# Zain-Jiang/Dict-TTS

Measured on AMD Instinct MI355X. Metric: mel-frames/sec, end-to-end text->mel->wav (audio-samples/sec = 256x; RTF reported alongside), higher is better.
Workload: dtype f16 (vocoder ResBlocks fp16 MFMA, serial convolutions bf16 hi/lo split; acoustic model fp32-grade: fp32 MFMA / bf16 three-piece operands x 6 products)

## Files before the change

dict_tts_amd/csrc/rb_common.h:

```cpp
#pragma once
#include <hip/hip_runtime.h>
#include <stdint.h>
#include "voc_el.h"

namespace dtts {

constexpr int VP_ST_AUX = 18;
constexpr int VP_LD_AUX = 18;
constexpr int VP_XI_AUX = 2;
constexpr int RB_X_AUX = 0;

typedef __attribute__((ext_vector_type(8))) __bf16 bf16x8;
typedef __attribute__((ext_vector_type(16))) float f32x16;
typedef __attribute__((ext_vector_type(4))) float f32x4;

__device__ __forceinline__ unsigned rf2bf(float f) {
    const __bf16 h = (__bf16)f;
    return (unsigned)__builtin_bit_cast(unsigned short, h);
}

typedef __attribute__((ext_vector_type(2))) float f32x2_t;
typedef __attribute__((ext_vector_type(2))) __bf16 bf16x2_t;
__device__ __forceinline__ unsigned pack2bf(float a, float b) {
    const bf16x2_t v = __builtin_convertvector(f32x2_t{a, b}, bf16x2_t);
// ... 226 lines not shown
            } else {
                xb += TU * dilP;
            }
        } else {
#pragma unroll
            for (int m = 0; m < MH * MT; ++m)
#pragma unroll
                for (int n = 0; n < NT; ++n) acc[m][n] = (*cinit)[n];
        }
    }
    for (; s0 < SG; s0 += 4) {
        const acc_t(&dummy)[NT] = *(const acc_t(*)[NT])acc[0];
        rb_group<EL, MT, NT, NKG, PITCH, false, MH, SH>(acc, dummy, ring, xa, act, wpf, xb, dilP, g);
        wpf += 4 * KGS;
        if constexpr (NKG >= 4) {
            if (++g == GPT) {
                g = 0;
                xb += dilP;
            }
        } else {
            xb += TU * dilP;
        }
    }
    if constexpr (TAIL) {
        const acc_t(&dummy)[NT] = *(const acc_t(*)[NT])acc[0];
        rb_group<EL, MT, NT, NKG, PITCH, false, MH, SH, 2>(acc, dummy, ring, xa, act, wpf, xb, dilP, 0);
    }
}

template <int NT, int RD>
__device__ __forceinline__ void rb2_preload(uint4 (&ring)[RD][NT], const uint4* w, int kgs) {
#pragma unroll
    for (int s = 0; s < RD - 1; ++s)
#pragma unroll
        for (int n = 0; n < NT; ++n) ring[s][n] = w[(size_t)s * kgs + n * 64];
}

template <int EL, int MT, int NT, int NKG, int PITCH, int RD, bool FIRST, bool CINIT>
__device__ __forceinline__ bool rb2_group(f32x16 (&acc)[MT][NT], const f32x16 (&cinit)[NT], uint4 (&ring)[RD][NT], uint4 (&xa)[MT],
                                          const char* act, const uint4* wpf, int xb, int dilP, int left) {
    constexpr int KGS = (NKG / 2) * 64;
    static_assert(RD % NKG == 0 && RD % 2 == 0, "a ring turn covers whole taps");
#pragma unroll
    for (int u = 0; u < RD; ++u) {
        if (u && u % NKG == 0 && u >= left) return true;
#pragma unroll
        for (int n = 0; n < NT; ++n) ring[(u + RD - 1) % RD][n] = wpf[u * KGS + n * 64];
        const int off = xb + ((u + 1) / NKG) * dilP + ((u + 1) % NKG) * 32;
        __builtin_amdgcn_sched_barrier(0);
#pragma unroll
        for (int m = 0; m < MT; ++m)
#pragma unroll
            for (int n = 0; n < NT; ++n) {
                if (FIRST && CINIT && u == 0) acc[m][n] = mfma16<EL>(ring[u][n], xa[m], cinit[n]);
                else acc[m][n] = mfma16<EL>(ring[u][n], xa[m], acc[m][n]);
                if (n == NT - 1) {
                    __builtin_amdgcn_sched_barrier(0);
                    xa[m] = *(const uint4*)(act + off + m * 32 * PITCH);
                    __builtin_amdgcn_sched_barrier(0);
                }
            }
        __builtin_amdgcn_sched_barrier(0);
    }
    return left <= RD;
}

template <int EL, int MT, int NT, int NKG, int PITCH, int RD, bool CINIT>
__device__ __forceinline__ void rb2_contract(f32x16 (&acc)[MT][NT], uint4 (&ring)[RD][NT], const char* act, int xrow0, const uint4* w, int S,
                                             int dilP, const f32x16 (&cinit)[NT]) {
    constexpr int KGS = (NKG / 2) * 64;
    uint4 xa[MT];
#pragma unroll
    for (int m = 0; m < MT; ++m) xa[m] = *(const uint4*)(act + xrow0 + m * 32 * PITCH);
    const uint4* wpf = w + (RD - 1) * KGS;
    int xb = xrow0;
    if (rb2_group<EL, MT, NT, NKG, PITCH, RD, true, CINIT>(acc, cinit, ring, xa, act, wpf, xb, dilP, S)) return;
    for (int left = S - RD;; left -= RD) {
        wpf += RD * KGS;
        xb += (RD / NKG) * dilP;
        if (rb2_group<EL, MT, NT, NKG, PITCH, RD, false, CINIT>(acc, cinit, ring, xa, act, wpf, xb, dilP, left)) return;
    }
}

}
```

dict_tts_amd/csrc/rblock.h:

```cpp
#pragma once
#include <hip/hip_runtime.h>
#include <stdint.h>
#include "voc_el.h"

namespace dtts {

struct RBlockParams {
    const float* x;
    float* S;
    unsigned short* Sa;
    struct Set {
        const uint4* w1[3];
        const uint4* w2[3];
        const float* b1[3];
        const float* b2[3];
        int dil[3];
        int K, Kp;
    } rb[3];
    int nrb;
    const int* lens;
    int B, T;
    int K;
    int mode;
    int last_mode;
    int drop_S;
    float div, slope;
    float* wav;
    const float* post_w;
    const float* post_b;
    int el;
    unsigned* tile_ctr;
    int pre_off;
    unsigned* bad;
    unsigned long long* ovf;
    int small_tile;
    int : 32;
    int s_private;
};

__host__ __device__ inline int rblock_halo_of(int K, const int* dil) {
    const int need = (K - 1) / 2 * (dil[0] + dil[1] + dil[2] + 3);
    return need > 6 * (K - 1) ? need : 6 * (K - 1);
}
__host__ __device__ inline int rblock_halo(const RBlockParams& p) {
    int h = 6 * (p.K - 1);
    for (int j = 0; j < p.nrb && j < 3; ++j) {
        const int need = rblock_halo_of(p.rb[j].K, p.rb[j].dil);
        h = need > h ? need : h;
    }
    return h;
}

constexpr int rblock_mfma_shape(int C) { return C == 64 ? 16 : 32; }

bool rblock_supported(int C, int K);
int rblock_padded_taps(int C, int K);
hipError_t rblock_launch(const RBlockParams& p, int C, int frag, hipStream_t stream);
long long rblock_private_rows(int C, int halo, int B, int T);
int rblock_stage_tile_rows(int C, int halo);
bool rblock_stage_launch_fits(int C, int halo, int B, bool wav);

}
```

dict_tts_amd/csrc/rblock.hip:

```cpp
#include "rblock.h"
#include "rb_common.h"

#include <algorithm>
#include <type_traits>
#include <cstdlib>

namespace dtts {

#ifdef RB_STAMP
__device__ unsigned long long rb_stamps[2][12][16];
extern "C" __attribute__((visibility("default"))) int dtts_debug_rb_stamps(unsigned long long* host, int reset) {
    hipError_t e = hipMemcpyFromSymbol(host, HIP_SYMBOL(rb_stamps), sizeof(rb_stamps));
    if (e == hipSuccess && reset) {
        static unsigned long long z[2][12][16];
        e = hipMemcpyToSymbol(HIP_SYMBOL(rb_stamps), z, sizeof z);
    }
    return (int)e;
}
#define RB_T(k) do { const unsigned long long _n = __builtin_amdgcn_s_memrealtime(); tq[k] += _n - t_last; t_last = _n; } while (0)
#else
#define RB_T(k)
#endif

template <int C, int MT, int NT, int WT, int WC, int EL, int PS, bool GUARD, bool TB = false, class SH = MfmaShape<32>>
// ... 53 lines not shown
    constexpr int RPP = THREADS / F4;
    constexpr int PER = SROWS / RPP;
    static_assert(THREADS % F4 == 0 && SROWS % RPP == 0, "row-coalesced staging");
    int c4 = tid % F4, r0 = tid / F4;
    auto tile_row = [&](int m, int u) { const int sr = r0 + RPP * u; return ((sr >> 5) * MT + m) * 32 + (sr & 31); };

    auto locate = [&](int jj, int& bb) {
        while (pre[bb + 1] <= jj) ++bb;
        bb = __builtin_amdgcn_readfirstlane(bb);
    };
    auto load_x = [&](acc_t (&d)[NT], int m, int bb, int base, int ln) {
        const auto rs = __builtin_amdgcn_make_buffer_rsrc((void*)(p.x + (long long)bb * p.T * C), 0, ln * C * 4, 0x00020000);
        const int o0 = ((base + wt * MT * 32 + SH::row(lane, 0)) * C + wc * NT * 32 + SH::chan(lane, 0)) * 4;
#pragma unroll
        for (int n = 0; n < NT; ++n)
#pragma unroll
            for (int q = 0; q < 4; ++q) {
                const u32x4 v = __builtin_amdgcn_raw_buffer_load_b128(rs, o0 + (m * 32 * C + n * 32 + SH::row(0, q) * C + SH::chan(0, q)) * 4, 0, RB_X_AUX);
                SH::set_quad(d[n], q, __builtin_bit_cast(f32x4, v));
            }
    };
    auto len_of = [&](int bb) { return __builtin_amdgcn_readfirstlane(pre[2 * p.B + 1 + bb]); };

    int b = 0, len, t0;
    if constexpr (PS) {
        locate(j, b);
        len = len_of(b);
        t0 = (j - pre[b]) * TTo - (p.wav ? PH : 0);
    } else {
        b = blockIdx.y;
        len = __builtin_amdgcn_readfirstlane(p.lens ? p.lens[b] : p.T);
        t0 = blockIdx.x * TTo - (p.wav ? PH : 0);
        if (t0 + (p.wav ? PH : 0) >= len) return;
    }
    acc_t xr[MT][NT];
    if constexpr (PS) {
#pragma unroll
        for (int m = 0; m < MT; ++m) load_x(xr[m], m, b, t0 - H, len);
    } else {
        const auto rs_x = __builtin_amdgcn_make_buffer_rsrc((void*)(p.x + (long long)b * p.T * C), 0, len * C * 4, 0x00020000);
        const int g0 = ((t0 - H + r0) * C + c4 * 4) * 4;
        u32x4 ld[MT][PER] = {};
#pragma unroll
        for (int m = 0; m < MT; ++m)
#pragma unroll
            for (int u = 0; u < PER; ++u) ld[m][u] = __builtin_amdgcn_raw_buffer_load_b128(rs_x, g0 + (tile_row(m, u) - r0) * (C * 4), 0, RB_X_AUX);
#pragma unroll
        for (int m = 0; m < MT; ++m) {
            if (m) __syncthreads();
#pragma unroll
            for (int u = 0; u < PER; ++u) *(u32x4*)(stage + (r0 + RPP * u) * EP + c4 * 16) = ld[m][u];
            __syncthreads();
#pragma unroll
            for (int n = 0; n < NT; ++n)
#pragma unroll
                for (int q = 0; q < 4; ++q)
                    SH::set_quad(xr[m][n], q, *(const f32x4*)(stage + (wt * 32 + SH::row(lane, q)) * EP + ((wc * NT + n) * 32 + SH::chan(lane, q)) * 4));
        }
    }

    const int kg_stride = (C / 32) * SH::WF * 64;
    int r = 0;

#ifdef RB_STAMP
    unsigned long long tq[16] = {0, 0, 0, 0, 0, 0, 0, 0, 0, 0, 0, 0, 0, 0, 0, 0};
    unsigned long long t_last = __builtin_amdgcn_s_memrealtime();
#endif
#pragma unroll 1
    for (;;) {
    if constexpr (PS) {
        tid = threadIdx.x;
        asm volatile("" : "+v"(tid));
        lane = tid & 63, wave = __builtin_amdgcn_readfirstlane(tid >> 6);
        wt = wave % WT, wc = wave / WT;
        c4 = tid % F4, r0 = tid / F4;
    }
    const int xlane = (RB_GUARD + wt * MT * 32 + SH::row(lane, 0)) * PITCH + SH::chan(lane, 0) * 4;
    const size_t wlane = (size_t)(wc * NT) * SH::WF * 64 + lane;
    if constexpr (PS) r = __builtin_amdgcn_readfirstlane(r);
    else r = 0;
    const RBlockParams::Set& R = p.rb[PS ? r : 0];
    const int Kr = R.K;
    constexpr bool REAL_STEPS = (C == 32);
    static_assert(!REAL_STEPS || SH::FRAG == 32, "rb2_contract is written for 32x32x16");
    static_assert(REAL_STEPS || NKG >= 4 || (NKG == 2 && SH::FRAG == 16), "whole groups of four k-steps, or rb_contract's half group");
    const int S = (REAL_STEPS ? Kr : R.Kp) * NKG;
    const bool last_rb = !PS || r + 1 == p.nrb;
    const int mode = (!PS || p.nrb == 1 || r == 0) ? p.mode : (last_rb ? p.last_mode : 1);
    const bool wav_now = p.wav && last_rb;
    t0 = __builtin_amdgcn_readfirstlane(t0);
    const int base_t = t0 - H;
    const long long brow = (long long)b * p.T;
    unsigned claim = 0;
    if (PS && p.tile_ctr && tid == 0 && last_rb) claim = atomicAdd(p.tile_ctr, 1u);
    int jn = j + G;
    bool has_next = PS && jn < total;
    int bn = b, lenn = len, t0n = 0;
    auto plan_next = [&]() {
        if (!last_rb) {
            has_next = true;
            jn = j;
            bn = b;
            lenn = len;
            t0n = t0;
            return;
        }
        has_next = PS && jn < total;
        bn = b;
        if (has_next) {
            locate(jn, bn);
            lenn = len_of(bn);
            t0n = (jn - pre[bn]) * TTo - (p.wav ? PH : 0);
        }
    };
    if (!(PS && p.tile_ctr) || !last_rb) plan_next();
    const auto rs_s = p.s_private ? __builtin_amdgcn_make_buffer_rsrc((void*)p.S, 0, p.s_private, 0x00020000)
                                  : __builtin_amdgcn_make_buffer_rsrc((void*)(p.S + brow * C), 0, len * C * 4, 0x00020000);

    constexpr int NBQ = 4 / SH::QB;
    auto load_bias = [&](f32x4 (&bb)[NT][NBQ], const float* bias) {
#pragma unroll
        for (int n = 0; n < NT; ++n)
#pragma unroll
            for (int q = 0; q < NBQ; ++q) bb[n][q] = *(const f32x4*)(bias + (wc * NT + n) * 32 + SH::chan(lane, q * SH::QB));
    };
    const bool all_inb = base_t >= 0 && base_t + W <= len;
    int n_ovf = 0;
    auto write_act_impl = [&](char* dst, const acc_t (&v)[MT][NT], auto masked_tag) {
        constexpr bool MASKED = decltype(masked_tag)::value;
        int ln = lane;
        if constexpr (SH::FRAG == 16) asm volatile("" : "+v"(ln));
#pragma unroll
        for (int m = 0; m < MT; ++m) {
            int row[SH::QB];
            bool inb[SH::QB], counted[SH::QB];
#pragma unroll
            for (int rh = 0; rh < SH::QB; ++rh) {
                row[rh] = (wt * MT + m) * 32 + SH::row(ln, rh);
                const int t = base_t + row[rh];
                inb[rh] = !MASKED || (t >= 0 && t < len);
                counted[rh] = inb[rh] && row[rh] >= H && row[rh] < H + TT;
            }
#pragma unroll
            for (int n = 0; n < NT; ++n)
#pragma unroll
                for (int q = 0; q < 4; ++q) {
                    constexpr int QBM = SH::QB - 1;
                    const int co = (wc * NT + n) * 32 + SH::chan(ln, q);
                    const f32x4 v4 = SH::quad(v[m][n], q);
                    uint2 pk = act4<EL>(v4, 0.1f);
                    if constexpr (GUARD) n_ovf += counted[q & QBM] ? ovf4(v4, 0.1f) : 0;
                    if constexpr (MASKED) {
                        if (!inb[q & QBM]) pk = make_uint2(0, 0);
                    }
                    *(uint2*)(dst + (RB_GUARD + row[q & QBM]) * PITCH + co * 2) = pk;
                }
        }
    };
    auto write_act = [&](char* dst, const acc_t (&v)[MT][NT]) {
        if (all_inb) write_act_impl(dst, v, std::false_type{});
        else write_act_impl(dst, v, std::true_type{});
    };

    uint4 ring[SH::RD][NT * SH::WF];
    f32x4 bb[NT][NBQ];
    RB_T(10);
    rb_preload(ring, R.w1[0] + wlane, kg_stride);
    load_bias(bb, R.b1[0]);
    write_act(act, xr);
    RB_T(0);
    __syncthreads();
    RB_T(1);

    acc_t acc[MT][NT];
#pragma unroll 1
    for (int it = 0; it < 3; ++it) {
        acc_t cinit[NT];
#pragma unroll
        for (int n = 0; n < NT; ++n)
#pragma unroll
            for (int q = 0; q < 4; ++q) SH::set_quad(cinit[n], q, bb[n][q / SH::QB]);
        load_bias(bb, R.b2[it]);
        const int d = R.dil[it];
        if constexpr (REAL_STEPS) {
            if (S) rb2_contract<EL, MT, NT, NKG, PITCH, 4, true>(acc, ring, act, xlane - ((Kr - 1) / 2) * d * PITCH, R.w1[it] + wlane, S, d * PITCH, cinit);
            else rb_contract<EL, MT, NT, NKG, PITCH, true, 1>(acc, ring, act, 0, R.w1[it] + wlane, 0, 0, &cinit);
        } else
            rb_contract<EL, MT, NT, NKG, PITCH, true, 1, SH>(acc, ring, act, xlane - ((Kr - 1) / 2) * d * PITCH, R.w1[it] + wlane, S, d * PITCH, &cinit);
        rb_preload(ring, R.w2[it] + wlane, kg_stride);
        RB_T(2);
        if constexpr (!TB) __syncthreads();
        RB_T(3);
        write_act(act2, acc);
        RB_T(4);
        __syncthreads();
        RB_T(5);
#pragma unroll
        for (int m = 0; m < MT; ++m)
#pragma unroll
            for (int n = 0; n < NT; ++n)
#pragma unroll
                for (int q = 0; q < 4; ++q) SH::add_quad(xr[m][n], q, bb[n][q / SH::QB]);
        if (it < 2) load_bias(bb, R.b1[it + 1]);
        if constexpr (REAL_STEPS) {
            if (S) rb2_contract<EL, MT, NT, NKG, PITCH, 4, false>(xr, ring, act2, xlane - ((Kr - 1) / 2) * PITCH, R.w2[it] + wlane, S, PITCH, cinit);
        } else
            rb_contract<EL, MT, NT, NKG, PITCH, false, 1, SH>(xr, ring, act2, xlane - ((Kr - 1) / 2) * PITCH, R.w2[it] + wlane, S, PITCH);
        if (it < 2) rb_preload(ring, R.w1[it + 1] + wlane, kg_stride);
        if (PS && p.tile_ctr && last_rb && it == 2 && tid == 0) pre[3 * p.B + 1] = G + (int)claim;
        RB_T(6);
        if (!TB || it == 2) __syncthreads();
        RB_T(7);
        if (it < 2) {
            write_act(act, xr);
            RB_T(0);
            __syncthreads();
            RB_T(1);
        }
    }

    if (PS && p.tile_ctr && last_rb) {
        jn = __builtin_amdgcn_readfirstlane(pre[3 * p.B + 1]);
        plan_next();
    }
    {
    const auto rs_a = __builtin_amdgcn_make_buffer_rsrc((void*)(p.Sa ? p.Sa + brow * C : (unsigned short*)(p.S + brow * C)), 0,
                                                        len * C * 2, 0x00020000);
    constexpr int CW = NT * 32, F4W = CW / 4, RPI = 64 / F4W, NRD = 32 / RPI;
    const int er = lane / F4W, ec = lane % F4W;
    const int goffw = (p.s_private ? (j * TT - H) * C : base_t * C) * 4 + (wc * CW + ec * 4) * 4;
    static_assert(F4W == 8 && RPI == 8 && NRD == 4, "the conflict-free row order below is for 8 lanes per row, 8 rows per access");
    const int erow_slab_base = C == 32 ? er : (er >> 2) + ((er & 1) ? 16 : 0) + ((er & 2) ? 8 : 0);
    auto srow = [&](int u) { return (C == 32 ? 8 : 2) * u + erow_slab_base; };
    auto erow = [&](int m, int u) { return (wt * MT + m) * 32 + srow(u); };
    auto eoff = [&](int m, int u) {
        const int row = erow(m, u);
        return (row >= H && row < H + TT) ? goffw + row * (C * 4) : (int)0x80000000;
    };
    u32x4 sold[MT][NRD];
#pragma unroll
    for (int m = 0; m < MT; ++m)
#pragma unroll
        for (int u = 0; u < NRD; ++u) {
            sold[m][u] = u32x4{0u, 0u, 0u, 0u};
            if (mode >= 1) sold[m][u] = p.nrb > 1 ? __builtin_amdgcn_raw_buffer_load_b128(rs_s, eoff(m, u), 0, 0)
                                                  : __builtin_amdgcn_raw_buffer_load_b128(rs_s, eoff(m, u), 0, VP_LD_AUX);
        }
    RB_T(12);
    constexpr int OP = C * 4;
    char* otile = smem;
    char* estage = wav_now ? smem + ((TB || (size_t)TT * OP > ACT_BYTES) ? (size_t)TT * OP : ACT_BYTES) : stage;
    char* stg = estage + (wt * 32) * EP + (wc * CW) * 4;
#pragma unroll
    for (int m = 0; m < MT; ++m) {
#pragma unroll
        for (int n = 0; n < NT; ++n)
#pragma unroll
            for (int q = 0; q < 4; ++q) *(f32x4*)(stg + SH::row(lane, q) * EP + (n * 32 + SH::chan(lane, q)) * 4) = SH::quad(xr[m][n], q);
        if (has_next) load_x(xr[m], m, bn, t0n - H, lenn);
        __builtin_amdgcn_fence(__ATOMIC_RELEASE, "wavefront");
        __builtin_amdgcn_wave_barrier();
        __builtin_amdgcn_fence(__ATOMIC_ACQUIRE, "wavefront");
        RB_T(13);
#pragma unroll
        for (int u = 0; u < NRD; ++u) {
            const int off = eoff(m, u);
            f32x4 o = *(const f32x4*)(stg + srow(u) * EP + ec * 16);
            o += __builtin_bit_cast(f32x4, sold[m][u]);
            if (wav_now) {
                const int row = erow(m, u);
                if (row >= H && row < H + TT) {
                    const int t = base_t + row;
#pragma unroll
                    for (int e = 0; e < 4; ++e) o[e] = (t >= 0 && t < len) ? lrelu(o[e] / p.div, p.slope) : 0.f;
                    *(f32x4*)(otile + (size_t)(row - H) * OP + (wc * CW + ec * 4) * 4) = o;
                }
                continue;
            }
            if (mode == 2) {
#pragma unroll
                for (int e = 0; e < 4; ++e) o[e] = o[e] / p.div;
            }
            if (!(mode == 2 && p.Sa && p.drop_S)) {
                if (p.nrb > 1 && !last_rb) __builtin_amdgcn_raw_buffer_store_b128(__builtin_bit_cast(u32x4, o), rs_s, off, 0, 0);
                else __builtin_amdgcn_raw_buffer_store_b128(__builtin_bit_cast(u32x4, o), rs_s, off, 0, VP_ST_AUX);
            }
            if (mode == 2 && p.Sa) {
// ... 97 lines not shown
static size_t rb_lds_bytes(int TT, bool wav) {
    constexpr int W = 32 * MT * WT, PITCH = C * 2 + 16, EP = C * 4 + 16;
    constexpr size_t ACT = (size_t)(W + 2 * RB_GUARD) * PITCH;
    if (wav)
        return TB ? std::max(2 * ACT, (size_t)TT * C * 4 + (size_t)WT * 32 * EP) : std::max((size_t)TT * C * 4, ACT) + (size_t)WT * 32 * EP;
    return TB ? std::max(2 * ACT, ACT + (size_t)RB_GUARD * PITCH + (size_t)WT * 32 * EP) : ACT + (size_t)WT * 32 * EP;
}
static size_t rb_table_bytes(int B) { return (size_t)(3 * B + 2) * sizeof(int); }

template <int C, int MT, int NT, int WT, int WC, int EL, int PS, bool GUARD = false, bool TB = false>
static hipError_t rb_launch_cfg(const RBlockParams& p, hipStream_t stream) {
    typedef MfmaShape<rblock_mfma_shape(C)> SH;
    constexpr int W = 32 * MT * WT;
    for (int j = 0; j < p.nrb; ++j)
        if (!(p.rb[j].K & 1) || p.rb[j].Kp != rblock_padded_taps(C, p.rb[j].K)) return hipErrorInvalidValue;
    const int H = rblock_halo(p), TT = W - 2 * H;
    if (TT < 32) return hipErrorInvalidValue;
    if ((long long)p.T * C * 4 >= (1LL << 31)) return hipErrorInvalidValue;
    if (p.wav && (C != 32 || (p.nrb == 1 && p.mode != 2) || !p.post_w || !p.post_b)) return hipErrorInvalidValue;
    size_t lds = rb_lds_bytes<C, MT, WT, TB>(TT, p.wav != nullptr);
    const int TTo = p.wav ? TT - 6 : TT;
    RBlockParams q = p;
    q.pre_off = (int)lds;
    if (PS) lds += rb_table_bytes(p.B);
    if (lds > 160 * 1024) return hipErrorOutOfMemory;
    constexpr bool HAS_GUARD = !(C == 64 && MT == 5);
    if constexpr (EL == EL_F16 && !GUARD && HAS_GUARD) {
        if (p.ovf) return rb_launch_cfg<C, MT, NT, WT, WC, EL, PS, true, TB>(p, stream);
    }
    if (EL == EL_F16 && !HAS_GUARD && p.ovf) return hipErrorInvalidValue;
    auto kern = rblock_kernel<C, MT, NT, WT, WC, EL, PS, GUARD, TB, SH>;
    static bool configured_dev[64] = {};
    int cur_dev = 0;
    (void)hipGetDevice(&cur_dev);
    bool& configured = configured_dev[cur_dev & 63];
    if (!configured) {
        hipError_t e = hipFuncSetAttribute((const void*)kern, hipFuncAttributeMaxDynamicSharedMemorySize, 160 * 1024);
        if (e != hipSuccess) return e;
        configured = true;
    }
    constexpr int THREADS = 64 * WT * WC;
    if (!PS) {
        hipLaunchKernelGGL(kern, dim3((p.T + TTo - 1) / TTo, p.B), dim3(THREADS), lds, stream, q);
        return hipGetLastError();
    }
    static int cus_dev[64] = {};
    int& cus = cus_dev[cur_dev & 63];
    if (!cus) {
        hipDeviceProp_t prop;
        if (hipGetDeviceProperties(&prop, cur_dev) != hipSuccess) return hipErrorInvalidDevice;
        cus = prop.multiProcessorCount;
    }
    const int per_cu = std::max(1, std::min({(int)(160 * 1024 / lds), 2048 / THREADS, THREADS <= 256 ? 2 : 1}));
    const long long max_tiles = (long long)p.B * ((p.T + TTo - 1) / TTo);
    const int grid = (int)std::min<long long>((long long)cus * per_cu, max_tiles);
    if (grid <= 0) return hipSuccess;
    hipLaunchKernelGGL(kern, dim3(grid), dim3(THREADS), lds, stream, q);
    return hipGetLastError();
}

bool rblock_supported(int C, int K) {
    if (!(K & 1) || K < 3 || K > 11) return false;
    return C == 32 || C == 64 || ((C == 128 || C == 256) && K == 3);
}

int rblock_stage_tile_rows(int C, int halo) {
    return (C == 32 ? 1024 : 512) - 2 * halo;
}

bool rblock_stage_launch_fits(int C, int halo, int B, bool wav) {
    const int TT = rblock_stage_tile_rows(C, halo);
    if (C != 32 && C != 64) return false;
    const size_t lds = (C == 32 ? rb_lds_bytes<32, 4, 8, false>(TT, wav) : rb_lds_bytes<64, 4, 4, false>(TT, wav)) + rb_table_bytes(B);
    return TT >= 32 && lds <= 160 * 1024;
}

long long rblock_private_rows(int C, int halo, int B, int T) {
    if (C != 32) return 0;
    const int TT = rblock_stage_tile_rows(C, halo), TTo = TT - 6;
    if (TTo < 32) return 0;
    return (long long)B * ((T + TTo - 1) / TTo) * TT;
}

int rblock_padded_taps(int C, int K) {
    const int sh = rblock_mfma_shape(C);
    const int nkg = C / (sh == 16 ? 32 : 16);
    if (sh == 16 && nkg == 2) return K;
    int kp = K;
    while ((kp * nkg) % 4) ++kp;
    return kp;
}

template <int EL>
static hipError_t rb_launch_el(const RBlockParams& p, int C, hipStream_t stream) {
    static int cus_dev[64] = {};
    int cur_dev = 0;
    (void)hipGetDevice(&cur_dev);
    int& cus = cus_dev[cur_dev & 63];
    if (!cus) {
        hipDeviceProp_t prop;
        cus = hipGetDeviceProperties(&prop, cur_dev) == hipSuccess ? prop.multiProcessorCount : 256;
    }
    auto few = [&](int W) {
        const int tt = W - 2 * rblock_halo(p) - (p.wav ? 6 : 0);
        return tt >= 32 && 2 * (long long)p.B * ((p.T + tt - 1) / tt) <= cus;
    };
    if (p.nrb < 1 || p.nrb > 3) return hipErrorInvalidValue;
    if (p.nrb > 1) {
        if (C == 32) return rb_launch_cfg<32, 4, 1, 8, 1, EL, 1>(p, stream);
        if (C == 64) return rb_launch_cfg<64, 4, 1, 4, 2, EL, 1>(p, stream);
        return hipErrorInvalidValue;
    }
#define RB_TRY(call)                                   \
    do {                                               \
        const hipError_t e_ = (call);                  \
        if (e_ != hipErrorOutOfMemory) return e_;      \
    } while (0)
    if (C == 32 && p.K >= 7 && !few(1024)) RB_TRY((rb_launch_cfg<32, 4, 1, 8, 1, EL, 1>(p, stream)));
    if (C == 64 && few(512)) return rb_launch_cfg<64, 4, 1, 2, 2, EL, 1>(p, stream);
    if (C == 128 && few(256)) return rb_launch_cfg<128, 4, 1, 1, 4, EL, 1>(p, stream);
    if (C == 256 && few(128)) return rb_launch_cfg<256, 2, 1, 1, 8, EL, 1>(p, stream);
    if (C == 32) return rb_launch_cfg<32, 4, 1, 4, 1, EL, 0>(p, stream);
    if (C == 64 && p.K >= 7 && !p.small_tile && !(EL == EL_F16 && p.ovf)) RB_TRY((rb_launch_cfg<64, 5, 1, 4, 2, EL, 1>(p, stream)));
    if (C == 64) RB_TRY((rb_launch_cfg<64, 4, 1, 4, 2, EL, 1>(p, stream)));
    if (C == 64) return rb_launch_cfg<64, 4, 1, 2, 2, EL, 1>(p, stream);
    if (C == 128) RB_TRY((rb_launch_cfg<128, 4, 1, 2, 4, EL, 1>(p, stream)));
    if (C == 128) return rb_launch_cfg<128, 4, 1, 1, 4, EL, 1>(p, stream);
    if (C == 256) RB_TRY((rb_launch_cfg<256, 4, 1, 1, 8, EL, 1>(p, stream)));
    if (C == 256) return rb_launch_cfg<256, 2, 1, 1, 8, EL, 1>(p, stream);
#undef RB_TRY
    return hipErrorInvalidValue;
}

hipError_t rblock_launch(const RBlockParams& p, int C, int frag, hipStream_t stream) {
    if (C != 32 && C != 64 && C != 128 && C != 256) return hipErrorInvalidValue;
    if (frag != rblock_mfma_shape(C)) return hipErrorInvalidValue;
    return p.el == EL_F16 ? rb_launch_el<EL_F16>(p, C, stream) : rb_launch_el<EL_BF16>(p, C, stream);
}

}
```

dict_tts_amd/csrc/vocoder.hip:

```cpp
#include "ctx.h"

using namespace dtts;

namespace {

bool vocoder_fp16_analysis(dtts_ctx* h, Need& need) {
    const dtts_config& c = h->cfg;
    const std::string v = "vocoder.";
    const int nk = c.n_resblock_kernels;
    std::vector<double> pt_wc[2], pt_m2[2];
    for (int pass = 0; pass < 2; ++pass) {
        const double M = pass;
        auto conv = [&](const std::string& base, const std::vector<double>& uin, const std::vector<double>& min, std::vector<double>& uout,
                        std::vector<double>& mout) -> bool {
            const HostTensor* w = folded_weight(h, need, base);
            const std::vector<float> b = bias_of(need, base);
            if (!w || b.empty() || w->shape.size() != 3) return false;
            const int co_n = (int)w->shape[0], ci_n = (int)w->shape[1], k_n = (int)w->shape[2];
            if ((int)uin.size() < ci_n) return false;
            uout.assign(co_n, 0.0);
            mout.assign(co_n, 0.0);
            for (int co = 0; co < co_n; ++co) {
                double su = std::fabs((double)b[co]), sm = (double)b[co] * b[co];
                for (int ci = 0; ci < ci_n; ++ci) {
// ... 15 lines not shown
        if (!conv(v + "conv_pre", u, m, u2, m2)) return false;
        u.swap(u2);
        m.swap(m2);
        for (int i = 0; i < c.n_upsamples; ++i) {
            const int r = c.upsample_rates[i], k_n = c.upsample_kernel_sizes[i], pad = (k_n - r) / 2;
            const HostTensor* w = folded_weight(h, need, v + "ups." + std::to_string(i));
            const std::vector<float> b = bias_of(need, v + "ups." + std::to_string(i));
            if (!w || b.empty() || w->shape.size() != 3 || (int)w->shape[2] != k_n) return false;
            const int ci_n = (int)w->shape[0], co_n = (int)w->shape[1];
            std::vector<double> ux(co_n, 0.0), mx(co_n, 0.0);
            for (int co = 0; co < co_n; ++co)
                for (int ph = 0; ph < r; ++ph) {
                    double su = std::fabs((double)b[co]), sm = (double)b[co] * b[co];
                    for (int ci = 0; ci < ci_n; ++ci) {
                        const float* pw = &w->f[((size_t)ci * co_n + co) * k_n];
                        double a1 = 0, a2 = 0;
                        for (int k = (ph + pad) % r; k < k_n; k += r) {
                            a1 += std::fabs((double)pw[k]);
                            a2 += (double)pw[k] * pw[k];
                        }
                        su += a1 * u[ci];
                        sm += a2 * 0.505 * m[ci];
                    }
                    ux[co] = std::max(ux[co], su);
                    mx[co] = std::max(mx[co], sm);
                }
            std::vector<double> us(co_n, 0.0), ms(co_n, 0.0);
            for (int j = 0; j < nk; ++j) {
                std::vector<double> x = ux, xm = mx, xt, xtm, y, ym, xa(co_n), xam(co_n);
                const std::string rb = v + "resblocks." + std::to_string(i * nk + j);
                for (int mth = 0; mth < (h->resblock2 ? 2 : 3); ++mth) {
                    for (int q = 0; q < co_n; ++q) {
                        pt_wc[pass].push_back(x[q]);
                        pt_m2[pass].push_back(xm[q]);
                        xa[q] = x[q];
                        xam[q] = 0.505 * xm[q];
                    }
                    if (h->resblock2) {
                        if (!conv(rb + ".convs." + std::to_string(mth), xa, xam, y, ym)) return false;
                    } else {
                        if (!conv(rb + ".convs1." + std::to_string(mth), xa, xam, xt, xtm)) return false;
                        for (int q = 0; q < co_n; ++q) {
                            pt_wc[pass].push_back(xt[q]);
                            pt_m2[pass].push_back(xtm[q]);
                            xtm[q] *= 0.505;
                        }
                        if (!conv(rb + ".convs2." + std::to_string(mth), xt, xtm, y, ym)) return false;
                    }
                    for (int q = 0; q < co_n; ++q) {
                        x[q] += y[q];
                        xm[q] += ym[q];
                    }
                }
                for (int q = 0; q < co_n; ++q) {
                    us[q] += x[q] / nk;
                    ms[q] += xm[q] / nk;
                }
            }
            u.swap(us);
            m.swap(ms);
        }
    }
    if (pt_wc[0].size() != pt_wc[1].size()) return false;
    double a_wc = 0, b_wc = 0, a_m2 = 0, b_m2 = 0;
    for (size_t q = 0; q < pt_wc[0].size(); ++q) {
        a_wc = std::max(a_wc, pt_wc[0][q]);
        b_wc = std::max(b_wc, pt_wc[1][q] - pt_wc[0][q]);
        a_m2 = std::max(a_m2, pt_m2[0][q]);
        b_m2 = std::max(b_m2, pt_m2[1][q] - pt_m2[0][q]);
    }
    h->wc_const = a_wc;
    h->wc_lin = b_wc;
    h->est_const = std::sqrt(a_m2);
    h->est_lin = std::sqrt(b_m2);
    return true;
}

bool pack_rb_fused(dtts_ctx* h, Need& need, PackedConv& L, int eng, const std::string& base, int ch, int k, int dil, int frag) {
    const HostTensor* w = folded_weight(h, need, base);
    std::vector<float> bias = bias_of(need, base);
    if (!w || bias.empty()) return false;
    const float* pw = w->f.data();
    const int slack = ch >= 64 ? 1 : 2;
    const bool ok = pack_conv(h, L, eng, ch, ch, frag == RBN_FRAG ? rbn_padded_taps(ch, k) : rblock_padded_taps(ch, k) + slack,
                              [=](int co, int ci, int tap) { return tap < k ? pw[((size_t)co * ch + ci) * k + tap] : 0.f; }, bias, dil, 1, 0, 0, -1, frag);
    L.K = k;
    return ok;
}

bool vpair_pack_fits(const PackedConv& L, int ch, int k) {
    return L.C_in == ch && L.C_out == ch && L.C_in_pad == ch && L.C_out_pad == ch && L.K == k && L.frag == vpair_mfma_shape(ch);
}
bool vpair_runs(const dtts_config& c, bool resblock2, int eng_rb, int ch, int k, int d0, int d1, int d2) {
    const bool fuse = c.vocoder_precision == DTTS_VOC_F16 || !c.vocoder_unfused;
    return fuse && !resblock2 && eng_rb != ENG_BF16X3 && !rblock_supported(ch, k) && vpair_supported(ch, k, d0) && vpair_supported(ch, k, d1) &&
           vpair_supported(ch, k, d2);
}

}

namespace dtts {

int build_vocoder(dtts_ctx* h) {
    Need need{h, ""};
    const dtts_config& c = h->cfg;
    if (c.vocoder_precision != DTTS_VOC_BF16 && c.vocoder_precision != DTTS_VOC_BF16X3 && c.vocoder_precision != DTTS_VOC_F16)
        return fail(h, DTTS_E_INVAL, "vocoder_precision %d is not one of DTTS_VOC_BF16 / _BF16X3 / _F16", c.vocoder_precision);
    if (c.vocoder_precision == DTTS_VOC_F16 && c.audio_num_mel_bins % 4)
        return fail(h, DTTS_E_INVAL, "DTTS_VOC_F16 needs audio_num_mel_bins %% 4 == 0 (got %d); use DTTS_VOC_BF16X3", c.audio_num_mel_bins);
    if (!h->ovf_dev) {
        if (!(h->ovf_dev = (unsigned long long*)dev_alloc(h, sizeof(unsigned long long))) || hipMemset(h->ovf_dev, 0, sizeof(unsigned long long)) != hipSuccess)
            return fail(h, DTTS_E_NOMEM, "range-guard counter");
    }
    if (!h->bad_dev) {
        if (!(h->bad_dev = (unsigned*)dev_alloc(h, sizeof(unsigned))) || hipMemset(h->bad_dev, 0, sizeof(unsigned)) != hipSuccess)
            return fail(h, DTTS_E_NOMEM, "overflow-detector counter");
        void* hp = nullptr;
        if (hipHostMalloc(&hp, 64, hipHostMallocDefault) != hipSuccess) return fail(h, DTTS_E_NOMEM, "overflow-detector host word");
        h->bad_host = (volatile unsigned*)hp;
        *h->bad_host = 0;
    }
    const int eng = c.vocoder_precision == DTTS_VOC_BF16 ? ENG_BF16 : ENG_BF16X3;
    const int eng_rb = c.vocoder_precision == DTTS_VOC_F16 ? ENG_F16 : eng;
    const std::string v = "vocoder.";
    bool ok = pack_plain(h, need, h->conv_pre, eng, v + "conv_pre", 1, 1, 3);
    h->ups.resize(c.n_upsamples);
    h->hop = 1;
    for (int i = 0; ok && i < c.n_upsamples; ++i) {
        const int u = c.upsample_rates[i], k = c.upsample_kernel_sizes[i];
        const bool h2 = c.vocoder_precision == DTTS_VOC_F16 && i == 1 && DTTS_TUNE(h, 8192) && (u * (c.upsample_initial_channel >> (i + 1))) % 256 == 0 &&
                        (c.upsample_initial_channel >> i) % 128 == 0;
        ok = ok && pack_transposed(h, need, h->ups[i], h2 ? ENG_F16 : eng, v + "ups." + std::to_string(i), u, (k - u) / 2);
        h->hop *= u;
    }
    const int nk = c.n_resblock_kernels;
    h->rb1.assign((size_t)c.n_upsamples * nk, {});
    h->rb2.assign((size_t)c.n_upsamples * nk, {});
    const bool rb2x = h->resblock2;
    for (int i = 0; ok && i < c.n_upsamples * nk; ++i) {
        const int j = i % nk, k = c.resblock_kernel_sizes[j], n = rb2x ? 2 : 3;
        const int ch = c.upsample_initial_channel >> (i / nk + 1);
        const std::string r = v + "resblocks." + std::to_string(i);
        const int* dl = c.resblock_dilation_sizes[j];
        const bool vp = vpair_runs(c, rb2x, eng_rb, ch, k, dl[0], dl[1], dl[2]);
        const int frag = vp ? vpair_mfma_shape(ch) : 32;
        h->rb1[i].resize(n);
        if (!rb2x) h->rb2[i].resize(3);
        for (int mth = 0; ok && mth < n; ++mth) {
            const int d = c.resblock_dilation_sizes[j][mth];
            ok = ok && pack_plain(h, need, h->rb1[i][mth], eng_rb, r + (rb2x ? ".convs." : ".convs1.") + std::to_string(mth), d, 1, (k * d - d) / 2, true, 0, frag);
            if (!rb2x) ok = ok && pack_plain(h, need, h->rb2[i][mth], eng_rb, r + ".convs2." + std::to_string(mth), 1, 1, (k - 1) / 2, true, 0, frag);
            if (ok && vp && !vpair_pack_fits(h->rb1[i][mth], ch, k))
                return fail(h, DTTS_E_INVAL, "%s%d: weight shape [%d, %d, %d] is not the configured [%d, %d, %d]", (r + ".convs1.").c_str(), mth, h->rb1[i][mth].C_out,
                            h->rb1[i][mth].C_in, h->rb1[i][mth].K, ch, ch, k);
            if (ok && vp && !vpair_pack_fits(h->rb2[i][mth], ch, k))
                return fail(h, DTTS_E_INVAL, "%s%d: weight shape [%d, %d, %d] is not the configured [%d, %d, %d]", (r + ".convs2.").c_str(), mth, h->rb2[i][mth].C_out,
                            h->rb2[i][mth].C_in, h->rb2[i][mth].K, ch, ch, k);
        }
    }
    h->rbf1.assign((size_t)c.n_upsamples * nk, {});
    h->rbf2.assign((size_t)c.n_upsamples * nk, {});
    for (int i = 0; ok && rb2x && eng_rb != ENG_BF16X3 && i < c.n_upsamples * nk; ++i) {
        const int j = i % nk, k = c.resblock_kernel_sizes[j];
        const int ch = c.upsample_initial_channel >> (i / nk + 1);
        const int d0 = c.resblock_dilation_sizes[j][0], d1 = c.resblock_dilation_sizes[j][1];
        if (!rb2x_supported(ch, k, d0, d1) || h->rb1[i][0].C_in_pad != ch || nk < 2) {
            if (eng_rb == ENG_F16)
// ... 185 lines not shown
        rp.lens = lout;
        rp.B = B;
        rp.T = Tcur;
        rp.mode = j == 0 ? 0 : (j == nk - 1 ? 2 : 1);
        rp.div = (float)nk;
        rp.slope = last_stage ? 0.01f : 0.1f;
        rp.Sa = exact ? nullptr : Sa;
        rp.drop_S = exact ? 0 : 1;
        if (last_stage && j_last == nk - 1 && h->post_w) {
            rp.wav = wav;
            rp.post_w = h->post_w;
            rp.post_b = h->post_b;
            rp.Sa = nullptr;
            post_done = true;
        }
        rp.el = el;
        rp.tile_ctr = n_ctr < N_CTR ? ctrs + n_ctr++ : nullptr;
        rp.ovf = (exact && h->guard_on) ? h->ovf_dev : nullptr;
        rp.bad = h->bad_dev;
    }

    int rblock(int j, int fuse_n) {
        if (nk == 1) return fail(h, DTTS_E_INVAL, "fused ResBlock path needs >= 2 resblock kernels");
        if (j > 0 && j < fuse_n) return DTTS_OK;
        const int j_last = j == 0 ? fuse_n - 1 : j;
        RBlockParams rp;
        whole_rb_params(rp, j, j_last);
        rp.nrb = j_last - j + 1;
        rp.last_mode = j_last == nk - 1 ? 2 : 1;
        int frag = 0;
        for (int jj = j; jj <= j_last; ++jj) {
            RBlockParams::Set& st = rp.rb[jj - j];
            const auto& g1 = h->rbf1[(size_t)i * nk + jj];
            const auto& g2 = h->rbf2[(size_t)i * nk + jj];
            st.K = g1[0].K;
            st.Kp = rblock_padded_taps(ch, g1[0].K);
            if (jj == j) frag = g1[0].frag;
            for (int mth = 0; mth < 3; ++mth)
                if (g1[mth].frag != frag || g2[mth].frag != frag) frag = 0;
            for (int mth = 0; mth < 3; ++mth) {
                st.w1[mth] = (const uint4*)g1[mth].w_hi;
                st.w2[mth] = (const uint4*)g2[mth].w_hi;
                st.b1[mth] = g1[mth].bias;
                st.b2[mth] = g2[mth].bias;
                st.dil[mth] = g1[mth].dil;
            }
            rp.K = std::max(rp.K, st.K);
        }
        if (rp.wav && fuse_n == nk) rp.s_private = (int)std::min<size_t>(s_cap_bytes, (size_t)INT_MAX);
        rp.small_tile = DTTS_TUNE(h, 16384) ? 1 : 0;
        if (h->debug_misorder) frag = frag == 16 ? 32 : 16;
        Timed tm(h, TV, s);
        LAUNCH(rblock_launch(rp, ch, frag, s));
        return DTTS_OK;
    }

    int rbn(int j) {
        const auto& g1 = h->rbf1[(size_t)i * nk + j];
        const auto& g2 = h->rbf2[(size_t)i * nk + j];
        RBnParams rp;
        whole_rb_params(rp, j, j);
        rp.K = g1[0].K;
        rp.Kp = rbn_padded_taps(ch, g1[0].K);
        int frag = g1[0].frag;
        for (int mth = 0; mth < 3; ++mth) {
            if (g1[mth].frag != frag || g2[mth].frag != frag) frag = 0;
            rp.w1[mth] = (const uint4*)g1[mth].w_hi;
            rp.w2[mth] = (const uint4*)g2[mth].w_hi;
            rp.b1[mth] = g1[mth].bias;
            rp.b2[mth] = g2[mth].bias;
            rp.dil[mth] = g1[mth].dil;
        }
        if (h->debug_misorder) frag = 16;
        Timed tm(h, TV, s);
        LAUNCH(rbn_launch(rp, ch, frag, s));
        return DTTS_OK;
    }

    int rb2x(int j) {
        const auto& fv = h->rbf1[(size_t)i * nk + j];
        RB2xParams rp;
        whole_rb_params(rp, j, j);
        rp.K = fv[0].K;
        rp.Kp = rblock_padded_taps(ch, fv[0].K);
        for (int m = 0; m < 2; ++m) {
            rp.w[m] = (const uint4*)fv[m].w_hi;
            rp.b[m] = fv[m].bias;
            rp.dil[m] = fv[m].dil;
        }
        Timed tm(h, TV, s);
        LAUNCH(rb2x_launch(rp, ch, s));
        return DTTS_OK;
    }

    int vpair(int j) {
        const auto& c1 = h->rb1[(size_t)i * nk + j];
        const auto& c2 = h->rb2[(size_t)i * nk + j];
        for (int mth = 0; mth < 3; ++mth)
            if (!vpair_pack_fits(c1[mth], ch, c1[0].K) || !vpair_pack_fits(c2[mth], ch, c1[0].K))
                return fail(h, DTTS_E_STATE, "resblock %d is not packed for vpair<%d>", i * nk + j, ch);
        const float* xin = Xf;
        for (int mth = 0; mth < 3; ++mth) {
            VPairParams vp;
            memset(&vp, 0, sizeof vp);
            vp.x = xin;
            vp.w1 = (const uint4*)c1[mth].w_hi;
            vp.w2 = (const uint4*)c2[mth].w_hi;
            vp.b1 = c1[mth].bias;
            vp.b2 = c2[mth].bias;
            vp.lens = lout;
            vp.B = B;
            vp.T = Tcur;
            vp.K = c1[mth].K;
            vp.dil = c1[mth].dil;
            vp.div = (float)nk;
            vp.slope = last_stage ? 0.01f : 0.1f;
            vp.el = el;
            vp.tile_ctr = n_ctr < N_CTR ? ctrs + n_ctr++ : nullptr;
            vp.ovf = (exact && h->guard_on) ? h->ovf_dev : nullptr;
            const bool s16 = exact && !DTTS_TUNE(h, 32768);
            vp.x16 = (s16 && mth > 0) ? 1 : 0;
            if (mth < 2) {
                vp.y = mth == 0 ? Rf : Rg;
                vp.mode = 1;
                vp.y16 = s16 ? 1 : 0;
            } else {
                vp.y = Sf;
                vp.mode = j == 0 ? 1 : (j == nk - 1 ? 3 : 2);
                vp.ya = exact ? nullptr : Sa;
                vp.drop_y = exact ? 0 : 1;
            }
            xin = vp.y;
            Timed tm(h, TV, s);
            LAUNCH(vpair_launch(vp, ch, s));
        }
        return DTTS_OK;
    }

    int convs(int j) {
        if (exact) return fail(h, DTTS_E_STATE, "DTTS_VOC_F16: resblock %d has no fused kernel", i * nk + j);
        const auto& c1 = h->rb1[(size_t)i * nk + j];
        if (c1[0].frag != 32) return fail(h, DTTS_E_STATE, "resblock %d is packed for vpair, not for the per-convolution kernels", i * nk + j);
        const int n = h->resblock2 ? 2 : 3;
        for (int mth = 0; mth < n; ++mth) {
            const bf* xa = mth == 0 ? Xa : Ra;
            if (!h->resblock2) {
                VConvParams p = vparams(c1[mth], xa, lout, B, Tcur);
                p.ldx = ch;
                p.ya = Ta;
                p.ldya = ch;
                p.slope = 0.1f;
                Timed tm(h, TV, s);
                LAUNCH(vconv_launch(p, s));
                xa = Ta;
            }
            VConvParams p = vparams(h->resblock2 ? c1[mth] : h->rb2[(size_t)i * nk + j][mth], xa, lout, B, Tcur);
            p.ldx = ch;
            p.res = mth == 0 ? Xf : Rf;
            p.ldres = ch;
            if (mth < n - 1) {
                p.yf = Rf;
                p.ldyf = ch;
                p.ya = Ra;
                p.ldya = ch;
                p.slope = 0.1f;
            } else {
                p.yf = Sf;
// ... 283 lines not shown
```

Baseline: 1.316 million.

## Use 16x16 MFMA shape for ResBlock widths 32-256 with new ring contraction

Switches the fused ResBlock kernel's MFMA fragment shape from 32x32 to 16x16 for channel widths 32, 128 and 256 (64 already used it). It adds a generic ring-buffered contraction (rbr_contract) for the C=32 real-step path under the 16-wide shape. Padded-tap computation is also parameterized by shape so packing matches the fragment used. The aim is better MFMA utilization or lower register pressure at these widths, at the cost of more instructions per k-step and different load/compute interleaving.

```diff
diff --git a/dict_tts_amd/csrc/rb_common.h b/dict_tts_amd/csrc/rb_common.h
--- a/dict_tts_amd/csrc/rb_common.h
+++ b/dict_tts_amd/csrc/rb_common.h
@@ -332,4 +332,61 @@
     }
 }
 
-}
+template <int EL, int MT, int NT, int NKG, int PITCH, bool FIRST, bool CINIT, class SH>
+__device__ __forceinline__ bool rbr_group(typename SH::acc_t (&acc)[MT][NT], const typename SH::acc_t (&cinit)[NT], uint4 (&ring)[SH::RD][NT * SH::WF],
+                                          uint4 (&xa)[MT], const char* act, const uint4* wpf, int xb, int dilP, int left) {
+    constexpr int RD = SH::RD, WF = SH::WF, KB = SH::KB;
+    constexpr int KGS = NKG * SH::CI * 2 * WF;
+    constexpr int NP = MT * SH::XF;
+    static_assert(RD % NKG == 0, "a ring turn covers whole taps");
+#pragma unroll
+    for (int u = 0; u < RD; ++u) {
+        if (u && u % NKG == 0 && u >= left) return true;
+#pragma unroll
+        for (int n = 0; n < NT * WF; ++n) ring[(u + RD - 1) % RD][n] = wpf[u * KGS + n * 64];
+        const int cur = xb + (u / NKG) * dilP + (u % NKG) * KB;
+        const int off = xb + ((u + 1) / NKG) * dilP + ((u + 1) % NKG) * KB;
+        __builtin_amdgcn_sched_barrier(0);
+#pragma unroll
+        for (int m = 0; m < MT; ++m)
+#pragma unroll
+            for (int n = 0; n < NT; ++n) {
+                const uint4* xf[SH::XF];
+#pragma unroll
+                for (int f = 0; f < SH::XF; ++f) xf[f] = &xa[(m * SH::XF + f) % MT];
+                if (FIRST && CINIT && u == 0) SH::template mma<EL>(acc[m][n], &ring[u % RD][n * WF], xf, cinit[n]);
+                else SH::template mma<EL>(acc[m][n], &ring[u % RD][n * WF], xf, acc[m][n]);
+                if (n == NT - 1) {
+                    __builtin_amdgcn_sched_barrier(0);
+#pragma unroll
+                    for (int f = 0; f < SH::XF; ++f) {
+                        const int p = m * SH::XF + f, pn = (p + MT) % NP;
+                        xa[p % MT] = *(const uint4*)(act + (p + MT < NP ? cur : off) + (pn / SH::XF * 32 + pn % SH::XF * SH::XROWS) * PITCH);
+                    }
+                    __builtin_amdgcn_sched_barrier(0);
+                }
+            }
+        __builtin_amdgcn_sched_barrier(0);
+    }
+    return left <= RD;
+}
+
+template <int EL, int MT, int NT, int NKG, int PITCH, bool CINIT, class SH>
+__device__ __forceinline__ void rbr_contract(typename SH::acc_t (&acc)[MT][NT], uint4 (&ring)[SH::RD][NT * SH::WF], const char* act, int xrow0, const uint4* w,
+                                             int S, int dilP, const typename SH::acc_t (&cinit)[NT]) {
+    constexpr int RD = SH::RD;
+    constexpr int KGS = NKG * SH::CI * 2 * SH::WF;
+    uint4 xa[MT];
+#pragma unroll
+    for (int p = 0; p < MT; ++p) xa[p] = *(const uint4*)(act + xrow0 + (p / SH::XF * 32 + p % SH::XF * SH::XROWS) * PITCH);
+    const uint4* wpf = w + (RD - 1) * KGS;
+    int xb = xrow0;
+    if (rbr_group<EL, MT, NT, NKG, PITCH, true, CINIT, SH>(acc, cinit, ring, xa, act, wpf, xb, dilP, S)) return;
+    for (int left = S - RD;; left -= RD) {
+        wpf += RD * KGS;
+        xb += (RD / NKG) * dilP;
+        if (rbr_group<EL, MT, NT, NKG, PITCH, false, CINIT, SH>(acc, cinit, ring, xa, act, wpf, xb, dilP, left)) return;
+    }
+}
+
+}
diff --git a/dict_tts_amd/csrc/rblock.h b/dict_tts_amd/csrc/rblock.h
--- a/dict_tts_amd/csrc/rblock.h
+++ b/dict_tts_amd/csrc/rblock.h
@@ -51,7 +51,18 @@
     return h;
 }
 
-constexpr int rblock_mfma_shape(int C) { return C == 64 ? 16 : 32; }
+#ifndef RBLOCK_SHAPE16_WIDTHS
+#define RBLOCK_SHAPE16_WIDTHS (32 | 64 | 128 | 256)
+#endif
+constexpr int rblock_mfma_shape(int C) { return (C == 32 || C == 64 || C == 128 || C == 256) && (C & (RBLOCK_SHAPE16_WIDTHS)) ? 16 : 32; }
+
+constexpr int rblock_padded_taps_of(int C, int K, int sh) {
+    const int nkg = C / (sh == 16 ? 32 : 16);
+    if (sh == 16 && nkg <= 2) return K;
+    int kp = K;
+    while ((kp * nkg) % 4) ++kp;
+    return kp;
+}
 
 bool rblock_supported(int C, int K);
 int rblock_padded_taps(int C, int K);
diff --git a/dict_tts_amd/csrc/rblock.hip b/dict_tts_amd/csrc/rblock.hip
--- a/dict_tts_amd/csrc/rblock.hip
+++ b/dict_tts_amd/csrc/rblock.hip
@@ -159,7 +159,6 @@
     const RBlockParams::Set& R = p.rb[PS ? r : 0];
     const int Kr = R.K;
     constexpr bool REAL_STEPS = (C == 32);
-    static_assert(!REAL_STEPS || SH::FRAG == 32, "rb2_contract is written for 32x32x16");
     static_assert(REAL_STEPS || NKG >= 4 || (NKG == 2 && SH::FRAG == 16), "whole groups of four k-steps, or rb_contract's half group");
     const int S = (REAL_STEPS ? Kr : R.Kp) * NKG;
     const bool last_rb = !PS || r + 1 == p.nrb;
@@ -259,7 +258,9 @@
             for (int q = 0; q < 4; ++q) SH::set_quad(cinit[n], q, bb[n][q / SH::QB]);
         load_bias(bb, R.b2[it]);
         const int d = R.dil[it];
-        if constexpr (REAL_STEPS) {
+        if constexpr (REAL_STEPS && SH::FRAG == 16) {
+            rbr_contract<EL, MT, NT, NKG, PITCH, true, SH>(acc, ring, act, xlane - ((Kr - 1) / 2) * d * PITCH, R.w1[it] + wlane, S, d * PITCH, cinit);
+        } else if constexpr (REAL_STEPS) {
             if (S) rb2_contract<EL, MT, NT, NKG, PITCH, 4, true>(acc, ring, act, xlane - ((Kr - 1) / 2) * d * PITCH, R.w1[it] + wlane, S, d * PITCH, cinit);
             else rb_contract<EL, MT, NT, NKG, PITCH, true, 1>(acc, ring, act, 0, R.w1[it] + wlane, 0, 0, &cinit);
         } else
@@ -279,7 +280,9 @@
 #pragma unroll
                 for (int q = 0; q < 4; ++q) SH::add_quad(xr[m][n], q, bb[n][q / SH::QB]);
         if (it < 2) load_bias(bb, R.b1[it + 1]);
-        if constexpr (REAL_STEPS) {
+        if constexpr (REAL_STEPS && SH::FRAG == 16) {
+            rbr_contract<EL, MT, NT, NKG, PITCH, false, SH>(xr, ring, act2, xlane - ((Kr - 1) / 2) * PITCH, R.w2[it] + wlane, S, PITCH, cinit);
+        } else if constexpr (REAL_STEPS) {
             if (S) rb2_contract<EL, MT, NT, NKG, PITCH, 4, false>(xr, ring, act2, xlane - ((Kr - 1) / 2) * PITCH, R.w2[it] + wlane, S, PITCH, cinit);
         } else
             rb_contract<EL, MT, NT, NKG, PITCH, false, 1, SH>(xr, ring, act2, xlane - ((Kr - 1) / 2) * PITCH, R.w2[it] + wlane, S, PITCH);
@@ -543,14 +546,7 @@
     return (long long)B * ((T + TTo - 1) / TTo) * TT;
 }
 
-int rblock_padded_taps(int C, int K) {
-    const int sh = rblock_mfma_shape(C);
-    const int nkg = C / (sh == 16 ? 32 : 16);
-    if (sh == 16 && nkg == 2) return K;
-    int kp = K;
-    while ((kp * nkg) % 4) ++kp;
-    return kp;
-}
+int rblock_padded_taps(int C, int K) { return rblock_padded_taps_of(C, K, rblock_mfma_shape(C)); }
 
 template <int EL>
 static hipError_t rb_launch_el(const RBlockParams& p, int C, hipStream_t stream) {
diff --git a/dict_tts_amd/csrc/vocoder.hip b/dict_tts_amd/csrc/vocoder.hip
--- a/dict_tts_amd/csrc/vocoder.hip
+++ b/dict_tts_amd/csrc/vocoder.hip
@@ -121,7 +121,7 @@
     if (!w || bias.empty()) return false;
     const float* pw = w->f.data();
     const int slack = ch >= 64 ? 1 : 2;
-    const bool ok = pack_conv(h, L, eng, ch, ch, frag == RBN_FRAG ? rbn_padded_taps(ch, k) : rblock_padded_taps(ch, k) + slack,
+    const bool ok = pack_conv(h, L, eng, ch, ch, frag == RBN_FRAG ? rbn_padded_taps(ch, k) : rblock_padded_taps_of(ch, k, frag) + slack,
                               [=](int co, int ci, int tap) { return tap < k ? pw[((size_t)co * ch + ci) * k + tap] : 0.f; }, bias, dil, 1, 0, 0, -1, frag);
     L.K = k;
     return ok;
@@ -473,7 +473,7 @@
         RB2xParams rp;
         whole_rb_params(rp, j, j);
         rp.K = fv[0].K;
-        rp.Kp = rblock_padded_taps(ch, fv[0].K);
+        rp.Kp = rblock_padded_taps_of(ch, fv[0].K, 32);
         for (int m = 0; m < 2; ++m) {
             rp.w[m] = (const uint4*)fv[m].w_hi;
             rp.b[m] = fv[m].bias;
```

Result: no change. 1.327 million, median of 6 (+0.9%).
